# DongSky/few-shot-vit

Hardware: AMD Instinct MI355X
Metric: episodes_per_sec_5way_5shot_visformer_s (higher is better)
Workload: dtype bf16; 1 GPU; BASELINE configs[1]: Visformer-S (visformer_micro_80) miniImageNet-shaped 5-way 5-shot episodic eval, 15 query/class, 80x80 fp32 NCHW episodes resident in HBM, procedural weights + calibrated BN; images_per_episode=100, encoder_chunk_images=12800, distinct_episode_batches=16, parallelism=episode-parallel x1, one all-reduce of accuracy stats, ranks_seen=1, per_rank_eps=4505.6

## Files before the change

### few-shot-vit_amd/csrc/stage1_w4.hip

```cpp
#include <stdlib.h>
#include <type_traits>

#include "lds_dma.h"
#include "kernels.h"

namespace FSVIT_NS {

namespace s1w {
constexpr int C1 = 128, HID = 256, CH = 64, RING = 128, XRING = 192, HALO = 21, KW2 = 320;
constexpr int XP = XRING * 16;
constexpr int RINGB = RING * 16;
constexpr int PITCH = RINGB + 16;
constexpr int XR = 0;
constexpr int H1R = XR + (C1 / 8) * XP;
constexpr int H2P = CH * 16;
constexpr int H2 = H1R + (HID / 8) * PITCH;
constexpr bool TABLE = gelu_tab::ON;
constexpr int TAB = H2 + (HID / 8) * H2P;
constexpr int TABC = TAB + 2 * gelu_tab::TN;
constexpr int LDS_BYTES = TAB + gelu_tab::BYTES;
}

typedef float f32x16w __attribute__((ext_vector_type(16)));

#define W4_IC(v) std::integral_constant<int, (v)>{}

__device__ __forceinline__ void w4_mfma(const u32x4& w, const u32x4& x, f32x16w& c) {
  asm volatile(FSVIT_MFMA_32x32x16 " %0, %1, %2, %0" : "+v"(c) : "a"(w), "v"(x));
}
__device__ __forceinline__ void w4_mfma_z(const u32x4& w, const u32x4& x, f32x16w& c) {
  asm volatile(FSVIT_MFMA_32x32x16 " %0, %1, %2, 0" : "=&v"(c) : "a"(w), "v"(x));
}
__device__ __forceinline__ void w4_mfma_vw(const u32x4& w, const u32x4& x, f32x16w& c) {
  asm volatile(FSVIT_MFMA_32x32x16 " %0, %1, %2, %0" : "+v"(c) : "v"(w), "v"(x));
}
__device__ __forceinline__ void w4_mfma_az(const u32x4& w, const u32x4& x, f32x16w& c) {
  asm volatile(FSVIT_MFMA_32x32x16 " %0, %1, %2, 0" : "=&v"(c) : "a"(w), "a"(x));
}
__device__ __forceinline__ void w4_bar() {
  asm volatile("s_waitcnt lgkmcnt(0)\n\ts_barrier" ::: "memory");
  __builtin_amdgcn_sched_barrier(0);
}

template <bool PIPE, bool SC>
__global__ __launch_bounds__(256, 1) void stage1_w4_kernel(const bf16* __restrict__ x, bf16* __restrict__ y, const bf16* __restrict__ w1,
                                                           const float* __restrict__ b1, const bf16* __restrict__ w2, const bf16* __restrict__ w3, int M,
                                                           int H, int W, int n_chunks, int chunks_per_wg) {
  using namespace s1w;
  extern __shared__ __attribute__((aligned(16))) unsigned char smem[];
  const int t = threadIdx.x, lane = t & 63, p = lane & 31, kh = lane >> 5;
  const int w = __builtin_amdgcn_readfirstlane(t >> 6);
  const int q0 = blockIdx.x * chunks_per_wg;
  int q1 = q0 + chunks_per_wg; q1 = q1 < n_chunks ? q1 : n_chunks;
  if (q0 >= q1) return;
  if (t < 4 * (HID / 8)) reinterpret_cast<unsigned*>(smem + H1R + (t >> 2) * PITCH + RINGB)[t & 3] = 0u;
  if constexpr (TABLE) gelu_tab::fill(smem + TAB, t, 256);

  const int cR = 16 * ((p >> 2) & 1) + 4 * (p >> 3) + (p & 3);
  constexpr int W3A = 9;
  u32x4 wf1[2][8], wf2[2][9][2], wf3[W3A];
  const bf16* const w3row = w3 + (size_t)(32 * w + cR) * HID + 8 * kh;
#pragma unroll
  for (int at = 0; at < 2; ++at)
#pragma unroll
    for (int ks = 0; ks < 8; ++ks) {
      bf16x8 v = __builtin_bit_cast(bf16x8, *reinterpret_cast<const u32x4*>(w1 + (size_t)(64 * w + 32 * at + cR) * C1 + 16 * ks + 8 * kh));
#pragma unroll
      for (int e = 0; e < 8; ++e) v[e] = (bf16)((float)v[e] * 0.125f);
      wf1[at][ks] = __builtin_bit_cast(u32x4, v);
    }
#pragma unroll
  for (int gi = 0; gi < 2; ++gi)
#pragma unroll
    for (int tp = 0; tp < 9; ++tp)
#pragma unroll
      for (int ks = 0; ks < 2; ++ks) wf2[gi][tp][ks] = *reinterpret_cast<const u32x4*>(w2 + (size_t)(64 * w + 32 * gi + cR) * KW2 + tp * 32 + 16 * ks + 8 * kh);
#pragma unroll
  for (int ks = 0; ks < W3A; ++ks) wf3[ks] = *reinterpret_cast<const u32x4*>(w3row + 16 * ks);
  u32x4 wb[2], ones;
  {
    const bf16 one = (bf16)1.0f;
    const unsigned o2 = (unsigned)__builtin_bit_cast(unsigned short, one) * 0x10001u;
    ones = kh == 0 ? u32x4{o2, 0u, 0u, 0u} : u32x4{0u, 0u, 0u, 0u};
#pragma unroll
    for (int at = 0; at < 2; ++at) {
      const float b = b1[64 * w + 32 * at + cR] * 0.125f;
      const bf16 hi = (bf16)b, lo = (bf16)(b - (float)hi);
      const unsigned v = (unsigned)__builtin_bit_cast(unsigned short, hi) | ((unsigned)__builtin_bit_cast(unsigned short, lo) << 16);
      wb[at] = kh == 0 ? u32x4{v, 0u, 0u, 0u} : u32x4{0u, 0u, 0u, 0u};
    }
  }
#pragma unroll
  for (int at = 0; at < 2; ++at)
#pragma unroll
    for (int ks = 0; ks < 8; ++ks) asm volatile("" : "+a"(wf1[at][ks]));
#pragma unroll
  for (int gi = 0; gi < 2; ++gi)
#pragma unroll
    for (int tp = 0; tp < 9; ++tp)
#pragma unroll
      for (int ks = 0; ks < 2; ++ks) asm volatile("" : "+a"(wf2[gi][tp][ks]));
#pragma unroll
  for (int ks = 0; ks < W3A; ++ks) asm volatile("" : "+a"(wf3[ks]));
  asm volatile("" : "+a"(wb[0]), "+a"(wb[1]), "+a"(ones));

  int sb = 0;
  auto xslot16 = [&](int d) {
    int s = sb + d;
    s += s < 0 ? XRING : 0;
    s -= s >= XRING ? XRING : 0;
    return s * 16;
  };
  u32x4 px[4];
  unsigned pxok = 0;
  auto gload = [&](int q, int d0) {
    pxok = 0;
#pragma unroll
    for (int u0 = 0; u0 < 4; ++u0) {
      const int u = t + 256 * u0, pp = (u & 7) + 8 * (u >> 7), c8 = (u >> 3) & 15;
      const long m = (long)q * CH + d0 + pp;
      const bool ok = m >= 0 && m < M;
      px[u0] = *reinterpret_cast<const u32x4*>(x + (size_t)(ok ? m : 0) * C1 + c8 * 8);
      pxok |= ok ? (1u << u0) : 0u;
    }
  };
  auto lstore = [&](int d0) {
#pragma unroll
    for (int u0 = 0; u0 < 4; ++u0) {
      const int u = t + 256 * u0, pp = (u & 7) + 8 * (u >> 7), c8 = (u >> 3) & 15;
      const u32x4 v = ((pxok >> u0) & 1u) ? px[u0] : u32x4{0u, 0u, 0u, 0u};
      *reinterpret_cast<u32x4*>(smem + XR + c8 * XP + xslot16(d0 + pp)) = v;
    }
  };

  const unsigned char* const xb = smem + XR + kh * XP;
  unsigned char* const h1w = smem + H1R + (8 * w + 2 * kh) * PITCH;
  const int h1r_off = H1R + (8 * w + kh) * PITCH;
  unsigned char* const h2w = smem + H2 + (8 * w + 2 * kh) * H2P + p * 16;
  const unsigned char* const h2b = smem + H2 + kh * H2P + p * 16;
  const unsigned char* const xres = smem + XR + (4 * w + 2 * kh) * XP;
  bf16* const yl = y + 32 * w + 16 * kh;
  const int HW = H * W;

  f32x16w acc1[2][2], acc2[2][2], acc3[2];
  auto conv1_mfma = [&](int d0) {
#pragma unroll
    for (int bt = 0; bt < 2; ++bt) {
      const int slot = xslot16(d0 + 32 * bt + p);
      w4_mfma_az(wb[0], ones, acc1[0][bt]);
      w4_mfma_az(wb[1], ones, acc1[1][bt]);
#pragma unroll
      for (int ks = 0; ks < 8; ++ks) {
        const u32x4 xf = *reinterpret_cast<const u32x4*>(xb + 2 * ks * XP + slot);
        w4_mfma(wf1[0][ks], xf, acc1[0][bt]);
        w4_mfma(wf1[1][ks], xf, acc1[1][bt]);
      }
    }
  };
  auto conv2_mfma = [&](int q, int bt) {
    const int m = q * CH + 32 * bt + p;
    const int rem = m % HW;
    const int oy = m < M ? rem / W : -4, ox = rem % W;
#pragma unroll
    for (int tp = 0; tp < 9; ++tp) {
      const int dy = tp / 3 - 1, dx = tp % 3 - 1;
      const bool ok = (unsigned)(oy + dy) < (unsigned)H && (unsigned)(ox + dx) < (unsigned)W;
      const unsigned char* base = smem + h1r_off + (ok ? ((m + dy * W + dx) & (RING - 1)) * 16 : RINGB);
#pragma unroll
      for (int ks = 0; ks < 2; ++ks)
#pragma unroll
        for (int gi = 0; gi < 2; ++gi) {
          const u32x4 hf = *reinterpret_cast<const u32x4*>(base + (4 * gi + 2 * ks) * PITCH);
          if (tp == 0 && ks == 0) w4_mfma_z(wf2[gi][tp][ks], hf, acc2[gi][bt]);
          else w4_mfma(wf2[gi][tp][ks], hf, acc2[gi][bt]);
        }
    }
  };
  auto res_init = [&]() {
#pragma unroll
    for (int bt = 0; bt < 2; ++bt)
#pragma unroll
      for (int o = 0; o < 2; ++o) {
        const bf16x8 r = __builtin_bit_cast(bf16x8, *reinterpret_cast<const u32x4*>(xres + o * XP + xslot16(-CH + 32 * bt + p)));
#pragma unroll
        for (int e = 0; e < 8; ++e) acc3[bt][8 * o + e] = SC ? (float)r[e] : (float)r[e] * 0.125f;
      }
  };
  auto conv3_mfma = [&]() {
    u32x4 wv[16 - W3A];
#pragma unroll
    for (int i = 0; i < 16 - W3A; ++i) wv[i] = *reinterpret_cast<const u32x4*>(w3row + 16 * (W3A + i));
    asm volatile("s_nop 3" : "+v"(acc3[0]), "+v"(acc3[1]));
#pragma unroll
    for (int bt = 0; bt < 2; ++bt)
#pragma unroll
      for (int ks = 0; ks < 16; ++ks) {
        const u32x4 hf = *reinterpret_cast<const u32x4*>(h2b + 2 * ks * H2P + 32 * bt * 16);
        if (ks < W3A) w4_mfma(wf3[ks], hf, acc3[bt]);
        else w4_mfma_vw(wv[ks - W3A], hf, acc3[bt]);
      }
  };
  auto store_out = [&](int q) {
#pragma unroll
    for (int bt = 0; bt < 2; ++bt) {
      const long m = (long)q * CH + 32 * bt + p;
#pragma unroll
      for (int o = 0; o < 2; ++o) {
        u32x4 v;
#pragma unroll
        for (int j = 0; j < 4; ++j) v[j] = SC ? pk2(acc3[bt][8 * o + 2 * j], acc3[bt][8 * o + 2 * j + 1]) : pk2(8.0f * acc3[bt][8 * o + 2 * j], 8.0f * acc3[bt][8 * o + 2 * j + 1]);
        if (m < M) *reinterpret_cast<u32x4*>(yl + (size_t)m * C1 + 8 * o) = v;
      }
    }
  };

  float gx[4][16][2], gu[4][16][2];
  unsigned gp[4][16];
  auto g_a1 = [&](int J, int k, const f32x16w& a) {
#pragma unroll
    for (int h = 0; h < 2; ++h) {
      gx[J][k][h] = a[2 * (k & 7) + h];
      asm("v_mul_f32_e64 %0, %1, %1 clamp" : "=v"(gu[J][k][h]) : "v"(gx[J][k][h]));
    }
  };
  auto g_a2 = [&](int J, int k) {
#pragma unroll
    for (int h = 0; h < 2; ++h) {
      float pp = fmaf(1.0153755e-3f * 32768.0f, gu[J][k][h], -1.0678257e-1f * 512.0f);
      pp = fmaf(pp, gu[J][k][h], -2.3011138f * 8.0f);
      gu[J][k][h] = gx[J][k][h] * pp;
    }
  };
  auto g_e = [&](int J, int k) {
#pragma unroll
    for (int h = 0; h < 2; ++h) gu[J][k][h] = __builtin_amdgcn_exp2f(gu[J][k][h]);
  };
  auto g_ba = [&](int J, int k) {
#pragma unroll
    for (int h = 0; h < 2; ++h) gu[J][k][h] = 1.0f + gu[J][k][h];
  };
  auto g_br = [&](int J, int k) {
#pragma unroll
    for (int h = 0; h < 2; ++h) gu[J][k][h] = __builtin_amdgcn_rcpf(gu[J][k][h]);
  };
  auto g_c = [&](int J, int k) { gp[J][k] = pk2(gx[J][k][0] * gu[J][k][0], gx[J][k][1] * gu[J][k][1]); };
  auto g_slot = [&](auto jt, auto numt, auto rt, const f32x16w& a0, const f32x16w& a1, auto dst) {
    constexpr int J = decltype(jt)::value, NUM = decltype(numt)::value, r = decltype(rt)::value;
    static_for<16>([&](auto kc) {
      constexpr int k = decltype(kc)::value, st = k * NUM / 4;
      if constexpr (r == st) g_a1(J, k, k < 8 ? a0 : a1);
      if constexpr (r == st + 1) g_a2(J, k);
      if constexpr (r == st + 2) g_e(J, k);
      if constexpr (r == st + 3) g_ba(J, k);
      if constexpr (r == st + 4) g_br(J, k);
      if constexpr (r == st + 5) {
        g_c(J, k);
        if constexpr ((k & 3) == 3) *reinterpret_cast<u32x4*>(dst(k >> 3, (k >> 2) & 1)) = u32x4{gp[J][k - 3], gp[J][k - 2], gp[J][k - 1], gp[J][k]};
      }
    });
  };
#ifndef W4_TJOBS
#define W4_TJOBS 0xf
#endif
#ifndef W4_PF
#define W4_PF 3
#endif
#ifndef W4_TLAT
#define W4_TLAT 4
#endif
  unsigned tc[4][16], ta[4][16], tm[4][16];
  unsigned ad0[4][16], ad1[4][16];
  const unsigned tabc = __builtin_amdgcn_readfirstlane((unsigned)(size_t)(__attribute__((address_space(3))) unsigned char*)smem + TABC);
  unsigned tl[4][16], th[4][16];
  auto t_slot = [&](auto jt, auto numt, auto rt, const f32x16w& a0, const f32x16w& a1, auto dst) {
    constexpr int J = decltype(jt)::value, NUM = decltype(numt)::value, r = decltype(rt)::value;
    static_for<16>([&](auto kc) {
      constexpr int k = decltype(kc)::value, st = k * NUM / 4;
      if constexpr (r == st) {
        const f32x16w& a = k < 8 ? a0 : a1;
        tc[J][k] = pk2(a[2 * (k & 7)], a[2 * (k & 7) + 1]);
        asm("" : "+v"(tc[J][k]));
      }
      if constexpr (r == st + 1) ta[J][k] = gelu_tab::rebase(tc[J][k]);
      if constexpr (r == st + 2) {
        tm[J][k] = gelu_tab::sign_mask(tc[J][k]);
        ta[J][k] = gelu_tab::clamp_top(ta[J][k]);
      }
      if constexpr (r == st + 3) gelu_tab::addresses(ta[J][k] ^ tm[J][k], tabc, ad0[J][k], ad1[J][k]);
      if constexpr (r == st + 4) {
        tl[J][k] = gelu_tab::gather(ad0[J][k]);
        th[J][k] = gelu_tab::gather(ad1[J][k]);
      }
      if constexpr (r == st + 4 + W4_TLAT) {
        gp[J][k] = tl[J][k] | (th[J][k] << 16);
        if constexpr ((k & 3) == 3) *reinterpret_cast<u32x4*>(dst(k >> 3, (k >> 2) & 1)) = u32x4{gp[J][k - 3], gp[J][k - 2], gp[J][k - 1], gp[J][k]};
      }
    });
  };
  auto gelu_slot = [&](auto jt, auto nt, auto nv, auto rt, const f32x16w& a0, const f32x16w& a1, auto dst) {
    if constexpr (TABLE && ((W4_TJOBS >> decltype(jt)::value) & 1)) t_slot(jt, nt, rt, a0, a1, dst);
    else g_slot(jt, nv, rt, a0, a1, dst);
  };
  typedef std::integral_constant<int, 0> J0;
  typedef std::integral_constant<int, 1> J1;
  typedef std::integral_constant<int, 2> J2;
  typedef std::integral_constant<int, 3> J3;
  typedef std::integral_constant<int, 6> N6;
  typedef std::integral_constant<int, 7> N7;
  typedef std::integral_constant<int, 8> N8;

  const int divW = (65536 + W - 1) / W;
  int remq[2], tms[2];
  unsigned long long rmk[2][3], cmk[2][3];
  typedef __attribute__((address_space(3))) const u32x4 lds_frag;
  typedef lds_frag* lds_frag_t;
  const int h1r_lds = h1r_off + (int)(size_t)(__attribute__((address_space(3))) unsigned char*)smem;
  const int zero_off = h1r_lds + RINGB;
  auto tap_setup = [&](int q, int bt) {
    const int m = q * CH + 32 * bt + p;
    const int oy = m < M ? (remq[bt] * divW) >> 16 : -4;
    const int ox = remq[bt] - ((remq[bt] * divW) >> 16) * W;
    tms[bt] = (m & (RING - 1)) * 16;
#pragma unroll
    for (int d = 0; d < 3; ++d) {
      rmk[bt][d] = __builtin_amdgcn_ballot_w64((unsigned)(oy + d - 1) < (unsigned)H);
      cmk[bt][d] = __builtin_amdgcn_ballot_w64((unsigned)(ox + d - 1) < (unsigned)W);
    }
  };
  auto tap_addr = [&](int bt, int tp) {
    const int dy = tp / 3 - 1, dx = tp % 3 - 1;
    const unsigned long long mk = rmk[bt][tp / 3] & cmk[bt][tp % 3];
    const int in = h1r_lds + ((tms[bt] + (dy * W + dx) * 16) & (RINGB - 1));
    int r;
    asm("v_cndmask_b32_e64 %0, %1, %2, %3" : "=v"(r) : "v"(zero_off), "v"(in), "s"(mk));
    return r;
  };
  auto rem_advance = [&](int bt) {
    remq[bt] += CH;
#pragma unroll
    for (int i = 0; i < 4; ++i) remq[bt] -= remq[bt] >= HW ? HW : 0;
  };

  auto gelu1 = [&](long P0, int bt) {
    const int slot = (int)((P0 + 32 * bt + p) & (RING - 1)) * 16;
    auto dst = [&](int at, int o) { return h1w + (4 * at + o) * PITCH + slot; };
    static_for<36 + W4_TLAT>([&](auto rc) {
      gelu_slot(J1{}, N8{}, N8{}, rc, acc1[0][bt], acc1[1][bt], dst);
      __builtin_amdgcn_sched_barrier(0);
    });
  };
  auto gelu2 = [&](int bt) {
    auto dst = [&](int gi, int o) { return h2w + (4 * gi + o) * H2P + 32 * bt * 16; };
    static_for<36 + W4_TLAT>([&](auto rc) {
      gelu_slot(J3{}, N8{}, N8{}, rc, acc2[0][bt], acc2[1][bt], dst);
      __builtin_amdgcn_sched_barrier(0);
    });
  };

  gload(q0, -HALO);
  __syncthreads();
  lstore(-HALO);
  gload(q0, -HALO + CH);
  __syncthreads();
  conv1_mfma(-HALO);
  asm volatile("s_nop 15\n\ts_nop 3" : "+v"(acc1[0][0]), "+v"(acc1[0][1]), "+v"(acc1[1][0]), "+v"(acc1[1][1]));
  gelu1((long)q0 * CH - HALO, 0);
  gelu1((long)q0 * CH - HALO, 1);
  lstore(-HALO + CH);
  if (q0 + 1 < q1) gload(q0, -HALO + 2 * CH);
  __syncthreads();

#define W4_STAMP(i) do { } while (0)
  auto body_pipe = [&](int q) {
    const long Pn = (long)q * CH - HALO + CH;
    const int sn0 = (int)((Pn + p) & (RING - 1)) * 16, sn1 = (int)((Pn + 32 + p) & (RING - 1)) * 16;
    const int xn0 = xslot16(CH - HALO + p), xn1 = xslot16(CH - HALO + 32 + p);
    auto h2dst1 = [&](int gi, int o) { return h2w + (4 * gi + o) * H2P + 32 * 16; };
    auto h2dst0 = [&](int gi, int o) { return h2w + (4 * gi + o) * H2P; };
    auto h1dst0 = [&](int at, int o) { return h1w + (4 * at + o) * PITCH + sn0; };
    auto h1dst1 = [&](int at, int o) { return h1w + (4 * at + o) * PITCH + sn1; };
    u32x4 wv[16 - W3A];
    {
      u32x4 xf[3], rr[4];
      xf[0] = *reinterpret_cast<const u32x4*>(xb + xn0);
      xf[1] = *reinterpret_cast<const u32x4*>(xb + 2 * XP + xn0);
      __builtin_amdgcn_sched_barrier(0);
      static_for<36>([&](auto mc) {
        constexpr int m = decltype(mc)::value, bt = m / 18, j = m % 18;
        if constexpr (j < 2) w4_mfma_az(wb[j], ones, acc1[j][bt]);
        else {
          constexpr int ks = (j - 2) >> 1, at = (j - 2) & 1, f = 8 * bt + ks;
          w4_mfma(wf1[at][ks], xf[f % 3], acc1[at][bt]);
          if constexpr (at == 1 && f + 3 < 16) {
            constexpr int f3 = f + 3;
            xf[f3 % 3] = *reinterpret_cast<const u32x4*>(xb + 2 * (f3 & 7) * XP + (f3 >> 3 ? xn1 : xn0));
          }
        }
        if constexpr (m == 0) {
          asm volatile("s_nop 15\n\ts_nop 3" : "+v"(acc2[0][1]), "+v"(acc2[1][1]));
          xf[2] = *reinterpret_cast<const u32x4*>(xb + 4 * XP + xn0);
        }
        if constexpr (m >= 1 && m <= 35) gelu_slot(J0{}, N7{}, N7{}, W4_IC(m - 1), acc2[0][1], acc2[1][1], h2dst1);
        if constexpr (m >= 28 && m < 32) {
          constexpr int i = m - 28, bt2 = i >> 1, o = i & 1;
          rr[i] = *reinterpret_cast<const u32x4*>(xres + o * XP + xslot16(-CH + 32 * bt2 + p));
        }
        if constexpr (m >= 36 - (16 - W3A)) wv[m - (36 - (16 - W3A))] = *reinterpret_cast<const u32x4*>(w3row + 16 * (W3A + m - (36 - (16 - W3A))));
        if constexpr (m >= 32) {
          constexpr int i = m - 32, bt2 = i >> 1, o = i & 1;
          const bf16x8 r = __builtin_bit_cast(bf16x8, rr[i]);
#pragma unroll
          for (int e = 0; e < 8; ++e) acc3[bt2][8 * o + e] = SC ? (float)r[e] : (float)r[e] * 0.125f;
        }
        __builtin_amdgcn_sched_barrier(0);
      });
    }
    W4_STAMP(0);
    w4_bar();
    W4_STAMP(1);
    lstore(2 * CH - HALO);
    {
      u32x4 hf[W4_PF + 1];
#pragma unroll
      for (int i = 0; i < W4_PF; ++i) hf[i] = *reinterpret_cast<const u32x4*>(h2b + 2 * i * H2P);
      __builtin_amdgcn_sched_barrier(0);
      static_for<32>([&](auto mc) {
        constexpr int m = decltype(mc)::value, bt = m >> 4, ks = m & 15;
        if constexpr (ks < W3A) w4_mfma(wf3[ks], hf[m % (W4_PF + 1)], acc3[bt]);
        else w4_mfma_vw(wv[ks - W3A], hf[m % (W4_PF + 1)], acc3[bt]);
        if constexpr (m + W4_PF < 32) hf[(m + W4_PF) % (W4_PF + 1)] = *reinterpret_cast<const u32x4*>(h2b + 2 * ((m + W4_PF) & 15) * H2P + ((m + W4_PF) >> 4) * 32 * 16);
        gelu_slot(J1{}, N6{}, N7{}, mc, acc1[0][0], acc1[1][0], h1dst0);
        __builtin_amdgcn_sched_barrier(0);
      });
    }
    W4_STAMP(2);
    {
      u32x4 hf[W4_PF + 1];
      int ta = tap_addr(0, 0), tb = tap_addr(0, 1);
#pragma unroll
      for (int i = 0; i < W4_PF; ++i) hf[i] = *(lds_frag_t)(size_t)(unsigned)(ta + (4 * (i & 1) + 2 * ((i >> 1) & 1)) * PITCH);
      __builtin_amdgcn_sched_barrier(0);
      static_for<36>([&](auto mc) {
        constexpr int m = decltype(mc)::value, tp = m >> 2, ks = (m >> 1) & 1, gi = m & 1;
        if constexpr (m < 2) w4_mfma_z(wf2[gi][0][0], hf[m % (W4_PF + 1)], acc2[gi][0]);
        else w4_mfma(wf2[gi][tp][ks], hf[m % (W4_PF + 1)], acc2[gi][0]);
        if constexpr (m + W4_PF < 36) {
          constexpr int m3 = m + W4_PF;
          if constexpr ((m3 & 3) == 0) ta = tb;
          hf[m3 % (W4_PF + 1)] = *(lds_frag_t)(size_t)(unsigned)(ta + (4 * (m3 & 1) + 2 * ((m3 >> 1) & 1)) * PITCH);
          if constexpr ((m3 & 3) == 2 && (m3 >> 2) + 1 < 9 && (m3 >> 2) >= 1) tb = tap_addr(0, (m3 >> 2) + 1);
        }
        gelu_slot(J2{}, N7{}, N8{}, mc, acc1[0][1], acc1[1][1], h1dst1);
        if constexpr (m == 4 || m == 10 || m == 16 || m == 22) {
          constexpr int i = (m - 4) / 6, bt = i >> 1, o = i & 1;
          const long mm = (long)(q - 1) * CH + 32 * bt + p;
          u32x4 v;
#pragma unroll
          for (int j = 0; j < 4; ++j) v[j] = SC ? pk2(acc3[bt][8 * o + 2 * j], acc3[bt][8 * o + 2 * j + 1]) : pk2(8.0f * acc3[bt][8 * o + 2 * j], 8.0f * acc3[bt][8 * o + 2 * j + 1]);
          if (mm < M) *reinterpret_cast<u32x4*>(yl + (size_t)mm * C1 + 8 * o) = v;
        }
        if constexpr (m == 28) tap_setup(q, 1);
        __builtin_amdgcn_sched_barrier(0);
      });
    }
    W4_STAMP(3);
    w4_bar();
    W4_STAMP(4);
    {
      u32x4 hf[W4_PF + 1];
      int ta = tap_addr(1, 0), tb = tap_addr(1, 1);
#pragma unroll
      for (int i = 0; i < W4_PF; ++i) hf[i] = *(lds_frag_t)(size_t)(unsigned)(ta + (4 * (i & 1) + 2 * ((i >> 1) & 1)) * PITCH);
      __builtin_amdgcn_sched_barrier(0);
      static_for<36>([&](auto mc) {
        constexpr int m = decltype(mc)::value, tp = m >> 2, ks = (m >> 1) & 1, gi = m & 1;
        if constexpr (m < 2) w4_mfma_z(wf2[gi][0][0], hf[m % (W4_PF + 1)], acc2[gi][1]);
        else w4_mfma(wf2[gi][tp][ks], hf[m % (W4_PF + 1)], acc2[gi][1]);
        if constexpr (m == 0) asm volatile("s_nop 15\n\ts_nop 3" : "+v"(acc2[0][0]), "+v"(acc2[1][0]));
        if constexpr (m + W4_PF < 36) {
          constexpr int m3 = m + W4_PF;
          if constexpr ((m3 & 3) == 0) ta = tb;
          hf[m3 % (W4_PF + 1)] = *(lds_frag_t)(size_t)(unsigned)(ta + (4 * (m3 & 1) + 2 * ((m3 >> 1) & 1)) * PITCH);
          if constexpr ((m3 & 3) == 2 && (m3 >> 2) + 1 < 9 && (m3 >> 2) >= 1) tb = tap_addr(1, (m3 >> 2) + 1);
        }
        if constexpr (m >= 1) gelu_slot(J3{}, N7{}, N8{}, W4_IC(m - 1), acc2[0][0], acc2[1][0], h2dst0);
        if constexpr (m == 20) gload(q, 3 * CH - HALO);
        if constexpr (m == 30) { rem_advance(0); rem_advance(1); }
        if constexpr (m == 32) tap_setup(q + 1, 0);
        __builtin_amdgcn_sched_barrier(0);
      });
      if constexpr (!(TABLE && ((W4_TJOBS >> 3) & 1))) g_slot(J3{}, N8{}, W4_IC(35), acc2[0][0], acc2[1][0], h2dst0);
    }
    W4_STAMP(5);
  };

  for (int q = q0; q <= q1; ++q, sb = sb + CH >= XRING ? sb + CH - XRING : sb + CH) {
    if constexpr (PIPE) {
      if (q > q0 && q + 2 < q1) {
        if (q == q0 + 1) {
#pragma unroll
          for (int bt = 0; bt < 2; ++bt) remq[bt] = (q * CH + 32 * bt + p) % HW;
          tap_setup(q, 0);
        }
        body_pipe(q);
        continue;
      }
    }
    const bool cur = q < q1, prev = q > q0;
    const long Pn = (long)q * CH - HALO + CH;
    if (prev) {
      asm volatile("s_nop 15\n\ts_nop 3" : "+v"(acc2[0][1]), "+v"(acc2[1][1]));
      gelu2(1);
      res_init();
    }
    __syncthreads();
    if (cur && q + 1 < q1) lstore(2 * CH - HALO);
    if (prev) {
      conv3_mfma();
      asm volatile("s_nop 15\n\ts_nop 3" : "+v"(acc3[0]), "+v"(acc3[1]));
      store_out(q - 1);
    }
    if (cur) {
      conv1_mfma(CH - HALO);
      asm volatile("s_nop 15\n\ts_nop 3" : "+v"(acc1[0][0]), "+v"(acc1[0][1]), "+v"(acc1[1][0]), "+v"(acc1[1][1]));
      gelu1(Pn, 0);
      gelu1(Pn, 1);
    }
    __syncthreads();
    if (cur) {
      if (q + 2 < q1) gload(q, 3 * CH - HALO);
      conv2_mfma(q, 0);
      asm volatile("s_nop 15\n\ts_nop 3" : "+v"(acc2[0][0]), "+v"(acc2[1][0]));
      gelu2(0);
      conv2_mfma(q, 1);
    }
  }
}

__global__ __launch_bounds__(256) void stage1_w4_prescale_kernel(const bf16* __restrict__ w, bf16* __restrict__ ws, int n) {
  for (int i = blockIdx.x * 256 + threadIdx.x; i < n; i += gridDim.x * 256) ws[i] = (bf16)((float)w[i] * 8.0f);
}
int launch_stage1_w4_prescale(const void* w, void* ws, int n, hipStream_t s) {
  if (n <= 0) return 0;
  hipLaunchKernelGGL(stage1_w4_prescale_kernel, dim3((n + 255) / 256 < 256 ? (n + 255) / 256 : 256), dim3(256), 0, s, (const bf16*)w, (bf16*)ws, n);
  return (int)hipGetLastError();
}

int launch_stage1_w4(const void* x, void* y, const void* w1, const float* b1, const void* w2, const void* w3, int B, int H, int W, hipStream_t s, const void* w3s) {
  const long Ml = (long)B * H * W;
  if (Ml <= 0) return 0;
  if (Ml >= (1L << 31) - 256 || W > 20 || H * W < 16) return (int)hipErrorInvalidValue;
  const int M = (int)Ml, n_chunks = (M + s1w::CH - 1) / s1w::CH;
  int wgs = n_chunks < 256 ? n_chunks : 256;
  const int cpw = (n_chunks + wgs - 1) / wgs;
  wgs = (n_chunks + cpw - 1) / cpw;
  const bool sc = w3s != nullptr;
  auto kern = sc ? stage1_w4_kernel<true, true> : stage1_w4_kernel<true, false>;
  hipError_t e = hipFuncSetAttribute((const void*)kern, hipFuncAttributeMaxDynamicSharedMemorySize, s1w::LDS_BYTES);
  if (e != hipSuccess) return (int)e;
  hipLaunchKernelGGL(kern, dim3(wgs), dim3(256), s1w::LDS_BYTES, s, (const bf16*)x, (bf16*)y, (const bf16*)w1, b1, (const bf16*)w2, (const bf16*)(sc ? w3s : w3), M, H, W, n_chunks, cpw);
  return (int)hipGetLastError();
}

}
```

Before: 4508 episodes/s.

## Use buffer loads/stores with hardware bounds and MFMA-based residual init in stage1 kernel

```diff
diff --git a/few-shot-vit_amd/csrc/stage1_w4.hip b/few-shot-vit_amd/csrc/stage1_w4.hip
--- a/few-shot-vit_amd/csrc/stage1_w4.hip
+++ b/few-shot-vit_amd/csrc/stage1_w4.hip
@@ -19,6 +19,11 @@
 constexpr int TAB = H2 + (HID / 8) * H2P;
 constexpr int TABC = TAB + 2 * gelu_tab::TN;
 constexpr int LDS_BYTES = TAB + gelu_tab::BYTES;
+#ifndef W4_MAX_PIXELS
+#define W4_MAX_PIXELS ((1L << 24) - 1024)
+#endif
+constexpr long MAX_PIXELS = W4_MAX_PIXELS;
+static_assert(MAX_PIXELS >= CH && MAX_PIXELS <= (1L << 24) - 1024, "32-bit offsets");
 }
 
 typedef float f32x16w __attribute__((ext_vector_type(16)));
@@ -33,6 +38,9 @@
 }
 __device__ __forceinline__ void w4_mfma_vw(const u32x4& w, const u32x4& x, f32x16w& c) {
   asm volatile(FSVIT_MFMA_32x32x16 " %0, %1, %2, %0" : "+v"(c) : "v"(w), "v"(x));
+}
+__device__ __forceinline__ void w4_mfma_vz(const u32x4& w, const u32x4& x, f32x16w& c) {
+  asm volatile(FSVIT_MFMA_32x32x16 " %0, %1, %2, 0" : "=&v"(c) : "v"(w), "v"(x));
 }
 __device__ __forceinline__ void w4_mfma_az(const u32x4& w, const u32x4& x, f32x16w& c) {
   asm volatile(FSVIT_MFMA_32x32x16 " %0, %1, %2, 0" : "=&v"(c) : "a"(w), "a"(x));
@@ -105,31 +113,27 @@
   asm volatile("" : "+a"(wb[0]), "+a"(wb[1]), "+a"(ones));
 
   int sb = 0;
-  auto xslot16 = [&](int d) {
-    int s = sb + d;
-    s += s < 0 ? XRING : 0;
-    s -= s >= XRING ? XRING : 0;
-    return s * 16;
-  };
+  auto xslot16 = [&](int d, int l16) {
+    const int k = (sb + (d % XRING + XRING) % XRING) * 16;
+    const unsigned a = (unsigned)(k + l16), b = (unsigned)(k - XRING * 16 + l16);
+    return (int)(a < b ? a : b);
+  };
+  const int p16 = p * 16, pp16 = ((t & 7) + 8 * (t >> 7)) * 16;
+  const __amdgpu_buffer_rsrc_t xrs = __builtin_amdgcn_make_buffer_rsrc(const_cast<bf16*>(x), 0, M * (C1 * 2), 0x00020000);
+  const __amdgpu_buffer_rsrc_t yrs = __builtin_amdgcn_make_buffer_rsrc(y, 0, M * (C1 * 2), 0x00020000);
   u32x4 px[4];
-  unsigned pxok = 0;
   auto gload = [&](int q, int d0) {
-    pxok = 0;
 #pragma unroll
     for (int u0 = 0; u0 < 4; ++u0) {
       const int u = t + 256 * u0, pp = (u & 7) + 8 * (u >> 7), c8 = (u >> 3) & 15;
-      const long m = (long)q * CH + d0 + pp;
-      const bool ok = m >= 0 && m < M;
-      px[u0] = *reinterpret_cast<const u32x4*>(x + (size_t)(ok ? m : 0) * C1 + c8 * 8);
-      pxok |= ok ? (1u << u0) : 0u;
+      px[u0] = __builtin_amdgcn_raw_buffer_load_b128(xrs, (unsigned)(q * CH + d0 + pp) * (unsigned)(C1 * 2) + c8 * 16, 0, 0);
     }
   };
   auto lstore = [&](int d0) {
 #pragma unroll
     for (int u0 = 0; u0 < 4; ++u0) {
-      const int u = t + 256 * u0, pp = (u & 7) + 8 * (u >> 7), c8 = (u >> 3) & 15;
-      const u32x4 v = ((pxok >> u0) & 1u) ? px[u0] : u32x4{0u, 0u, 0u, 0u};
-      *reinterpret_cast<u32x4*>(smem + XR + c8 * XP + xslot16(d0 + pp)) = v;
+      const int u = t + 256 * u0, c8 = (u >> 3) & 15;
+      *reinterpret_cast<u32x4*>(smem + XR + c8 * XP + xslot16(d0 + 16 * u0, pp16)) = px[u0];
     }
   };
 
@@ -138,15 +142,26 @@
   const int h1r_off = H1R + (8 * w + kh) * PITCH;
   unsigned char* const h2w = smem + H2 + (8 * w + 2 * kh) * H2P + p * 16;
   const unsigned char* const h2b = smem + H2 + kh * H2P + p * 16;
-  const unsigned char* const xres = smem + XR + (4 * w + 2 * kh) * XP;
-  bf16* const yl = y + 32 * w + 16 * kh;
+  const unsigned char* const xres = smem + XR + (4 * w + kh) * XP;
+  const unsigned yoff = (32 * w + 16 * kh) * 2;
   const int HW = H * W;
+  u32x4 idf[2];
+  {
+    const bf16 iv = (bf16)(SC ? 1.0f : 0.125f);
+    const unsigned i1 = __builtin_bit_cast(unsigned short, iv);
+#pragma unroll
+    for (int j = 0; j < 2; ++j) {
+      const int e = cR - 16 * j - 8 * kh;
+#pragma unroll
+      for (int i = 0; i < 4; ++i) idf[j][i] = (e >> 1) == i ? i1 << (16 * (e & 1)) : 0u;
+    }
+  }
 
   f32x16w acc1[2][2], acc2[2][2], acc3[2];
   auto conv1_mfma = [&](int d0) {
 #pragma unroll
     for (int bt = 0; bt < 2; ++bt) {
-      const int slot = xslot16(d0 + 32 * bt + p);
+      const int slot = xslot16(d0 + 32 * bt, p16);
       w4_mfma_az(wb[0], ones, acc1[0][bt]);
       w4_mfma_az(wb[1], ones, acc1[1][bt]);
 #pragma unroll
@@ -176,21 +191,19 @@
         }
     }
   };
-  auto res_init = [&]() {
-#pragma unroll
-    for (int bt = 0; bt < 2; ++bt)
-#pragma unroll
-      for (int o = 0; o < 2; ++o) {
-        const bf16x8 r = __builtin_bit_cast(bf16x8, *reinterpret_cast<const u32x4*>(xres + o * XP + xslot16(-CH + 32 * bt + p)));
-#pragma unroll
-        for (int e = 0; e < 8; ++e) acc3[bt][8 * o + e] = SC ? (float)r[e] : (float)r[e] * 0.125f;
-      }
-  };
-  auto conv3_mfma = [&]() {
+  auto res_read = [&](u32x4 (&rr)[4]) {
+#pragma unroll
+    for (int i = 0; i < 4; ++i) rr[i] = *reinterpret_cast<const u32x4*>(xres + 2 * (i & 1) * XP + xslot16(-CH + 32 * (i >> 1), p16));
+  };
+  auto conv3_mfma = [&](const u32x4 (&rr)[4]) {
     u32x4 wv[16 - W3A];
 #pragma unroll
     for (int i = 0; i < 16 - W3A; ++i) wv[i] = *reinterpret_cast<const u32x4*>(w3row + 16 * (W3A + i));
-    asm volatile("s_nop 3" : "+v"(acc3[0]), "+v"(acc3[1]));
+#pragma unroll
+    for (int bt = 0; bt < 2; ++bt) {
+      w4_mfma_vz(idf[0], rr[2 * bt], acc3[bt]);
+      w4_mfma_vw(idf[1], rr[2 * bt + 1], acc3[bt]);
+    }
 #pragma unroll
     for (int bt = 0; bt < 2; ++bt)
 #pragma unroll
@@ -203,13 +216,13 @@
   auto store_out = [&](int q) {
 #pragma unroll
     for (int bt = 0; bt < 2; ++bt) {
-      const long m = (long)q * CH + 32 * bt + p;
+      const unsigned mo = (unsigned)(q * CH + 32 * bt + p) * (unsigned)(C1 * 2) + yoff;
 #pragma unroll
       for (int o = 0; o < 2; ++o) {
         u32x4 v;
 #pragma unroll
         for (int j = 0; j < 4; ++j) v[j] = SC ? pk2(acc3[bt][8 * o + 2 * j], acc3[bt][8 * o + 2 * j + 1]) : pk2(8.0f * acc3[bt][8 * o + 2 * j], 8.0f * acc3[bt][8 * o + 2 * j + 1]);
-        if (m < M) *reinterpret_cast<u32x4*>(yl + (size_t)m * C1 + 8 * o) = v;
+        __builtin_amdgcn_raw_buffer_store_b128(v, yrs, mo + 16 * o, 0, 0);
       }
     }
   };
@@ -305,9 +318,16 @@
   typedef std::integral_constant<int, 1> J1;
   typedef std::integral_constant<int, 2> J2;
   typedef std::integral_constant<int, 3> J3;
-  typedef std::integral_constant<int, 6> N6;
   typedef std::integral_constant<int, 7> N7;
   typedef std::integral_constant<int, 8> N8;
+#ifndef W4_S2_NT
+#define W4_S2_NT 7
+#endif
+#ifndef W4_S2_NV
+#define W4_S2_NV 8
+#endif
+  typedef std::integral_constant<int, W4_S2_NT> W4_S2NT;
+  typedef std::integral_constant<int, W4_S2_NV> W4_S2NV;
 
   const int divW = (65536 + W - 1) / W;
   int remq[2], tms[2];
@@ -318,8 +338,11 @@
   const int zero_off = h1r_lds + RINGB;
   auto tap_setup = [&](int q, int bt) {
     const int m = q * CH + 32 * bt + p;
-    const int oy = m < M ? (remq[bt] * divW) >> 16 : -4;
-    const int ox = remq[bt] - ((remq[bt] * divW) >> 16) * W;
+    unsigned rm = (unsigned)(remq[bt] + p);
+#pragma unroll
+    for (int i = 0; i < 2; ++i) rm = rm < rm - (unsigned)HW ? rm : rm - (unsigned)HW;
+    const int oy = m < M ? ((int)rm * divW) >> 16 : -4;
+    const int ox = (int)rm - (((int)rm * divW) >> 16) * W;
     tms[bt] = (m & (RING - 1)) * 16;
 #pragma unroll
     for (int d = 0; d < 3; ++d) {
@@ -373,15 +396,17 @@
 #define W4_STAMP(i) do { } while (0)
   auto body_pipe = [&](int q) {
     const long Pn = (long)q * CH - HALO + CH;
-    const int sn0 = (int)((Pn + p) & (RING - 1)) * 16, sn1 = (int)((Pn + 32 + p) & (RING - 1)) * 16;
-    const int xn0 = xslot16(CH - HALO + p), xn1 = xslot16(CH - HALO + 32 + p);
+    const int pn16 = (int)(Pn & (RING - 1)) * 16;
+    const int sn0 = (pn16 + p16) & (RINGB - 1), sn1 = (pn16 + 32 * 16 + p16) & (RINGB - 1);
+    const int xn0 = xslot16(CH - HALO, p16), xn1 = xslot16(CH - HALO + 32, p16);
     auto h2dst1 = [&](int gi, int o) { return h2w + (4 * gi + o) * H2P + 32 * 16; };
     auto h2dst0 = [&](int gi, int o) { return h2w + (4 * gi + o) * H2P; };
     auto h1dst0 = [&](int at, int o) { return h1w + (4 * at + o) * PITCH + sn0; };
     auto h1dst1 = [&](int at, int o) { return h1w + (4 * at + o) * PITCH + sn1; };
     u32x4 wv[16 - W3A];
+    u32x4 rr[4];
     {
-      u32x4 xf[3], rr[4];
+      u32x4 xf[3];
       xf[0] = *reinterpret_cast<const u32x4*>(xb + xn0);
       xf[1] = *reinterpret_cast<const u32x4*>(xb + 2 * XP + xn0);
       __builtin_amdgcn_sched_barrier(0);
@@ -401,17 +426,11 @@
           xf[2] = *reinterpret_cast<const u32x4*>(xb + 4 * XP + xn0);
         }
         if constexpr (m >= 1 && m <= 35) gelu_slot(J0{}, N7{}, N7{}, W4_IC(m - 1), acc2[0][1], acc2[1][1], h2dst1);
-        if constexpr (m >= 28 && m < 32) {
-          constexpr int i = m - 28, bt2 = i >> 1, o = i & 1;
-          rr[i] = *reinterpret_cast<const u32x4*>(xres + o * XP + xslot16(-CH + 32 * bt2 + p));
+        if constexpr (m >= 32) {
+          constexpr int i = m - 32;
+          rr[i] = *reinterpret_cast<const u32x4*>(xres + 2 * (i & 1) * XP + xslot16(-CH + 32 * (i >> 1), p16));
         }
         if constexpr (m >= 36 - (16 - W3A)) wv[m - (36 - (16 - W3A))] = *reinterpret_cast<const u32x4*>(w3row + 16 * (W3A + m - (36 - (16 - W3A))));
-        if constexpr (m >= 32) {
-          constexpr int i = m - 32, bt2 = i >> 1, o = i & 1;
-          const bf16x8 r = __builtin_bit_cast(bf16x8, rr[i]);
-#pragma unroll
-          for (int e = 0; e < 8; ++e) acc3[bt2][8 * o + e] = SC ? (float)r[e] : (float)r[e] * 0.125f;
-        }
         __builtin_amdgcn_sched_barrier(0);
       });
     }
@@ -424,12 +443,18 @@
 #pragma unroll
       for (int i = 0; i < W4_PF; ++i) hf[i] = *reinterpret_cast<const u32x4*>(h2b + 2 * i * H2P);
       __builtin_amdgcn_sched_barrier(0);
-      static_for<32>([&](auto mc) {
-        constexpr int m = decltype(mc)::value, bt = m >> 4, ks = m & 15;
-        if constexpr (ks < W3A) w4_mfma(wf3[ks], hf[m % (W4_PF + 1)], acc3[bt]);
-        else w4_mfma_vw(wv[ks - W3A], hf[m % (W4_PF + 1)], acc3[bt]);
-        if constexpr (m + W4_PF < 32) hf[(m + W4_PF) % (W4_PF + 1)] = *reinterpret_cast<const u32x4*>(h2b + 2 * ((m + W4_PF) & 15) * H2P + ((m + W4_PF) >> 4) * 32 * 16);
-        gelu_slot(J1{}, N6{}, N7{}, mc, acc1[0][0], acc1[1][0], h1dst0);
+      static_for<36>([&](auto mc) {
+        constexpr int m = decltype(mc)::value;
+        if constexpr (m < 4) {
+          if constexpr (m < 2) w4_mfma_vz(idf[0], rr[2 * m], acc3[m]);
+          else w4_mfma_vw(idf[1], rr[2 * (m - 2) + 1], acc3[m - 2]);
+        } else {
+          constexpr int c = m - 4, bt = c >> 4, ks = c & 15;
+          if constexpr (ks < W3A) w4_mfma(wf3[ks], hf[c % (W4_PF + 1)], acc3[bt]);
+          else w4_mfma_vw(wv[ks - W3A], hf[c % (W4_PF + 1)], acc3[bt]);
+          if constexpr (c + W4_PF < 32) hf[(c + W4_PF) % (W4_PF + 1)] = *reinterpret_cast<const u32x4*>(h2b + 2 * ((c + W4_PF) & 15) * H2P + ((c + W4_PF) >> 4) * 32 * 16);
+        }
+        gelu_slot(J1{}, W4_S2NT{}, W4_S2NV{}, mc, acc1[0][0], acc1[1][0], h1dst0);
         __builtin_amdgcn_sched_barrier(0);
       });
     }
@@ -453,11 +478,11 @@
         gelu_slot(J2{}, N7{}, N8{}, mc, acc1[0][1], acc1[1][1], h1dst1);
         if constexpr (m == 4 || m == 10 || m == 16 || m == 22) {
           constexpr int i = (m - 4) / 6, bt = i >> 1, o = i & 1;
-          const long mm = (long)(q - 1) * CH + 32 * bt + p;
+          const unsigned mo = (unsigned)((q - 1) * CH + 32 * bt + p) * (unsigned)(C1 * 2) + yoff;
           u32x4 v;
 #pragma unroll
           for (int j = 0; j < 4; ++j) v[j] = SC ? pk2(acc3[bt][8 * o + 2 * j], acc3[bt][8 * o + 2 * j + 1]) : pk2(8.0f * acc3[bt][8 * o + 2 * j], 8.0f * acc3[bt][8 * o + 2 * j + 1]);
-          if (mm < M) *reinterpret_cast<u32x4*>(yl + (size_t)mm * C1 + 8 * o) = v;
+          __builtin_amdgcn_raw_buffer_store_b128(v, yrs, mo + 16 * o, 0, 0);
         }
         if constexpr (m == 28) tap_setup(q, 1);
         __builtin_amdgcn_sched_barrier(0);
@@ -499,7 +524,7 @@
       if (q > q0 && q + 2 < q1) {
         if (q == q0 + 1) {
 #pragma unroll
-          for (int bt = 0; bt < 2; ++bt) remq[bt] = (q * CH + 32 * bt + p) % HW;
+          for (int bt = 0; bt < 2; ++bt) remq[bt] = (q * CH + 32 * bt) % HW;
           tap_setup(q, 0);
         }
         body_pipe(q);
@@ -507,16 +532,17 @@
       }
     }
     const bool cur = q < q1, prev = q > q0;
+    u32x4 rr[4];
     const long Pn = (long)q * CH - HALO + CH;
     if (prev) {
       asm volatile("s_nop 15\n\ts_nop 3" : "+v"(acc2[0][1]), "+v"(acc2[1][1]));
       gelu2(1);
-      res_init();
+      res_read(rr);
     }
     __syncthreads();
     if (cur && q + 1 < q1) lstore(2 * CH - HALO);
     if (prev) {
-      conv3_mfma();
+      conv3_mfma(rr);
       asm volatile("s_nop 15\n\ts_nop 3" : "+v"(acc3[0]), "+v"(acc3[1]));
       store_out(q - 1);
     }
@@ -550,16 +576,26 @@
   const long Ml = (long)B * H * W;
   if (Ml <= 0) return 0;
   if (Ml >= (1L << 31) - 256 || W > 20 || H * W < 16) return (int)hipErrorInvalidValue;
-  const int M = (int)Ml, n_chunks = (M + s1w::CH - 1) / s1w::CH;
-  int wgs = n_chunks < 256 ? n_chunks : 256;
-  const int cpw = (n_chunks + wgs - 1) / wgs;
-  wgs = (n_chunks + cpw - 1) / cpw;
   const bool sc = w3s != nullptr;
   auto kern = sc ? stage1_w4_kernel<true, true> : stage1_w4_kernel<true, false>;
   hipError_t e = hipFuncSetAttribute((const void*)kern, hipFuncAttributeMaxDynamicSharedMemorySize, s1w::LDS_BYTES);
   if (e != hipSuccess) return (int)e;
-  hipLaunchKernelGGL(kern, dim3(wgs), dim3(256), s1w::LDS_BYTES, s, (const bf16*)x, (bf16*)y, (const bf16*)w1, b1, (const bf16*)w2, (const bf16*)(sc ? w3s : w3), M, H, W, n_chunks, cpw);
-  return (int)hipGetLastError();
-}
-
-}
+  int gcd = H * W, r = s1w::CH;
+  while (r) { const int tmp = gcd % r; gcd = r; r = tmp; }
+  const int align = s1w::CH / gcd;
+  const long fit = s1w::MAX_PIXELS / ((long)H * W) / align * align;
+  if (fit <= 0) return (int)hipErrorInvalidValue;
+  for (long b0 = 0; b0 < B; b0 += fit) {
+    const int M = (int)((B - b0 < fit ? B - b0 : fit) * H * W), n_chunks = (M + s1w::CH - 1) / s1w::CH;
+    int wgs = n_chunks < 256 ? n_chunks : 256;
+    const int cpw = (n_chunks + wgs - 1) / wgs;
+    wgs = (n_chunks + cpw - 1) / cpw;
+    const size_t off = (size_t)b0 * H * W * s1w::C1;
+    hipLaunchKernelGGL(kern, dim3(wgs), dim3(256), s1w::LDS_BYTES, s, (const bf16*)x + off, (bf16*)y + off, (const bf16*)w1, b1, (const bf16*)w2, (const bf16*)(sc ? w3s : w3), M, H, W, n_chunks, cpw);
+    e = hipGetLastError();
+    if (e != hipSuccess) return (int)e;
+  }
+  return 0;
+}
+
+}
```

New measurement: 4527 episodes/s, median of 6. No clear change (+0.4%).
